# soedinglab/MMseqs2

Measured on AMD Instinct MI355X. Metric: sw_gcells_per_s, higher is better.
Workload: dtype int16

## Files before the change

### mmseqs2_amd/csrc/mmgpu_api.hip

```cpp
#include <algorithm>
#include <atomic>
#include <thread>
#include <cmath>
#include <cstdio>
#include <cstring>
#include <numeric>
#include <string>
#include <vector>

#include "mmgpu_internal.h"

#include <chrono>

using namespace mmgpu;

namespace mmgpu {
thread_local std::string g_last_error;
}
using mmgpu::g_last_error;

extern "C" const char *mmgpu_last_error(void) { return g_last_error.c_str(); }

extern "C" int mmgpu_init(mmgpu_ctx **out, int device_id) {
    if (!out) return fail(MMGPU_ERR_ARG, "mmgpu_init: ctx is NULL");
// ... 594 lines not shown
        hit_out.resize((size_t)total_hits);
    }
    b->h_qout_off.assign(nq + 1, 0);
    if (mode >= MMGPU_SW_START && !pf) b->h_out_target.resize((size_t)total_hits);
    return MMGPU_OK;
}

int SwPrepare::copy_query(uint32_t i, int *qminp) {
    const mmgpu_sw_query &Q = qs[i];
    memcpy(qres.data() + qoff[i], Q.q, Q.qlen);
    int mincb = 0;
    *qminp = minp;
    for (uint32_t k = 0; k < Q.qlen; k++) {
        if (Q.q[k] >= par->alphabet) return fail(MMGPU_ERR_ARG, "mmgpu_sw_prepare: query residue code >= alphabet");
        if (Q.comp_bias && !Q.profile) { qcb[qoff[i] + k] = Q.comp_bias[k]; mincb = std::min<int>(mincb, Q.comp_bias[k]); }
    }
    if (Q.profile) {
        if (Q.profile_letters == 0 || (int)Q.profile_letters > par->alphabet)
            return fail(MMGPU_ERR_ARG, "mmgpu_sw_prepare: profile_letters must be in [1, alphabet]");
        if (qprof.size() + (size_t)par->alphabet * Q.qlen > 0xFFFFFFF0ull) return fail(MMGPU_ERR_UNSUPPORTED, "mmgpu_sw_prepare: more than 4 GB of query profiles in one batch");
        qprof_off[i] = (uint32_t)qprof.size();
        qprof.resize(qprof.size() + (size_t)par->alphabet * Q.qlen, 0);
        const uint32_t rows = std::min<uint32_t>(Q.profile_letters, (uint32_t)par->alphabet - 1);
        memcpy(qprof.data() + qprof_off[i], Q.profile, (size_t)rows * Q.qlen);
        *qminp = 0;
        for (size_t k = 0; k < (size_t)Q.profile_letters * Q.qlen; k++) *qminp = std::min<int>(*qminp, Q.profile[k]);
        b->any_profile = true;
        b->h_query_is_profile.resize(nq, 0);
        b->h_query_is_profile[i] = 1;
    }
    if (!(*qminp + mincb + par->gap_extend > -par->gap_open))
        return fail(MMGPU_ERR_UNSUPPORTED, "mmgpu_sw_prepare: gap penalties too small for this matrix (adjacent insertion+deletion could win)");
    qbias[i] = std::abs(*qminp) + std::abs(mincb);
    qminstart[i] = Q.min_start_score;
    return MMGPU_OK;
}

void SwPrepare::add_rev_jobs(uint32_t query, uint32_t first, uint32_t n, uint32_t shape, uint64_t cells_per_hit) {
    uint64_t per = 6 * JOB_CELLS / std::max<uint64_t>(cells_per_hit, 1);
    per = std::min<uint64_t>(std::max<uint64_t>(per / JOB_ROUND * JOB_ROUND, JOB_ROUND), (uint64_t)SW_REV_JOB_MAX);
    for (uint32_t k = 0; k < n; k += (uint32_t)per) {
        SwJob j;
        j.query = query;
        j.hit_begin = first + k;
        j.hit_end = first + std::min<uint32_t>(k + (uint32_t)per, n);
        j.shape = shape;
        rev_jobs.push_back(j);
        rev_cells.push_back(cells_per_hit * (j.hit_end - j.hit_begin) * 65536u + (n - k));
    }
}

void SwPrepare::add_slot_jobs(uint32_t i, uint32_t shape, uint32_t round, bool multi) {
    const mmgpu_sw_query &Q = qs[i];
    const uint64_t est_cells = (uint64_t)Q.qlen * ((Q.qlen + c->mean_len) / 2 + 1) * round;
    const uint32_t per_job = job_slots(round, JOB_CELLS / est_cells);
    for (uint32_t k = 0; k < pf_stride; k += per_job) {
        SwJob j;
        j.query = i;
        j.hit_begin = hit_cursor + k;
        j.hit_end = hit_cursor + std::min<uint32_t>(k + per_job, pf_stride);
        j.shape = shape | (multi ? n_multi++ << 8 : 0u);
        jobs.push_back(j);
        job_cells.push_back((uint64_t)Q.qlen * (j.hit_end - j.hit_begin) * 65536u + (pf_stride - k));
    }
    if (multi && mode >= MMGPU_SW_START)
        add_rev_jobs(i, hit_cursor, pf_stride, shape, (uint64_t)Q.qlen * ((Q.qlen + c->mean_len) / 2 + 1));
    max_tlen = c->db.max_len;
}

int SwPrepare::copy_queries() {
    for (uint32_t i = 0; i < nq; i++) {
        const mmgpu_sw_query &Q = qs[i];
        if (Q.qlen == 0) {
            b->h_qout_off[i + 1] = out_cursor;
            continue;
        }
        int qminp;
        if (int e = copy_query(i, &qminp)) return e;
        int rpl; bool multi;
        pick_class(Q.qlen, &rpl, &multi);
        any_multi |= multi;
        const uint32_t shape = (multi ? 32u : 0u) + (uint32_t)rpl - 1;
        const int grp = sw_shape_group(shape);
        b->group_lds[grp] = std::max(b->group_lds[grp], sw_lds_bytes(rpl, par->alphabet));
        const uint32_t round = (multi && Q.qlen >= LONG_QUERY) ? JOB_ROUND / 4 : JOB_ROUND;
        const uint32_t n_slots = pf ? pf_stride : Q.n_targets;
        if (pf) add_slot_jobs(i, shape, round, multi);
        else deferred.push_back(Deferred{i, hit_cursor, out_cursor, shape, round, multi});
        hit_cursor += n_slots;
        out_cursor += n_slots;
        b->h_qout_off[i + 1] = out_cursor;
    }
    return MMGPU_OK;
}

void SwPrepare::cut_list_jobs_of(size_t from, size_t to) {
    std::vector<uint32_t> ord;
    for (size_t d = from; d < to; d++) {
        const Deferred &D = deferred[d];
        const mmgpu_sw_query &Q = qs[D.query];
        PerQuery &P = per_query[d];
        const bool same_list = d > from && Q.target_ids == qs[deferred[d - 1].query].target_ids && Q.n_targets == qs[deferred[d - 1].query].n_targets;
        if (!same_list) {
            ord.resize(Q.n_targets);
            std::iota(ord.begin(), ord.end(), 0u);
            for (uint32_t k = 0; k < Q.n_targets; k++)
                if (Q.target_ids[k] >= c->db.n) { P.bad = true; break; }
            if (P.bad) continue;
            std::stable_sort(ord.begin(), ord.end(), [&](uint32_t a, uint32_t bb) {
                return c->h_len[Q.target_ids[a]] > c->h_len[Q.target_ids[bb]];
            });
        }
        for (uint32_t k = 0; k < Q.n_targets; k++) {
            const uint32_t t = Q.target_ids[ord[k]];
            hit_target[D.hit_cursor + k] = t;
            hit_out[D.hit_cursor + k] = D.out_cursor + ord[k];
            P.sum_cells += (uint64_t)Q.qlen * c->h_len[t];
            P.max_tlen = std::max(P.max_tlen, c->h_len[t]);
        }
        for (uint32_t k = 0; k < Q.n_targets;) {
            uint64_t jc = 0;
            uint32_t e = k;
            while (e < Q.n_targets && e - k < JOB_HITS) {
                const uint32_t stop = std::min<uint32_t>(e + D.round, Q.n_targets);
                for (; e < stop; e++) jc += (uint64_t)Q.qlen * c->h_len[hit_target[D.hit_cursor + e]];
                const uint32_t held = e - k;
                if (jc >= JOB_CELLS && (held <= 16 || held % JOB_ROUND == 0)) break;
            }
            SwJob j;
            j.query = D.query;
            j.hit_begin = D.hit_cursor + k;
            j.hit_end = D.hit_cursor + e;
            j.shape = D.shape;
            P.jobs.push_back(j);
            P.cells.push_back(jc);
            k = e;
        }
        if (Q.n_targets) P.rev_mid_len = c->h_len[hit_target[D.hit_cursor + Q.n_targets / 2]];
        if (mode >= MMGPU_SW_START)
            for (uint32_t k = 0; k < Q.n_targets; k++) b->h_out_target[D.out_cursor + k] = Q.target_ids[k];
    }
}

void SwPrepare::cut_list_jobs() {
    per_query.resize(deferred.size());
    static const unsigned host_threads = std::min(16u, std::max(1u, std::thread::hardware_concurrency()));
    const size_t n_thr = std::max<size_t>(1, std::min<size_t>(host_threads, total_hits / 65536 + 1));
    if (n_thr <= 1) {
        cut_list_jobs_of(0, deferred.size());
        return;
    }
    std::vector<std::thread> pool;
    size_t from = 0;
    uint64_t acc = 0;
    const uint64_t share = total_hits / n_thr + 1;
    for (size_t d = 0; d < deferred.size(); d++) {
        acc += qs[deferred[d].query].n_targets;
        if (acc >= share || d + 1 == deferred.size()) {
            pool.emplace_back(&SwPrepare::cut_list_jobs_of, this, from, d + 1);
            from = d + 1;
            acc = 0;
        }
    }
    for (std::thread &t : pool) t.join();
}

int SwPrepare::join_list_jobs() {
// ... 290 lines not shown
    S.n_slots = (uint32_t)slots;
    S.full = b->o_full.as<mmgpu_sw_hit>();
    S.status = b->o_status.as<uint32_t>();
    HIP_TRY(launch_sw_owned_scatter(S, c->stream));
    return MMGPU_OK;
}

}

extern "C" int mmgpu_sw_gather_owned(mmgpu_ctx *c, mmgpu_sw_batch_t *b, const void **d_full, const void **d_status) {
    if (!c || !b) return fail(MMGPU_ERR_ARG, "mmgpu_sw_gather_owned: NULL argument");
    const int n = c->comm ? c->comm->n_ranks : 1;
    for (int attempt = 0; attempt < 2; attempt++) {
        mmgpu::XchgBlock blk[2];
        if (int e = mmgpu::sw_gather_begin(c, b, n, blk)) return e;
        for (int k = 0; k < 2; k++)
            if (int e = mmgpu::comm_allgather(c, blk[k].send, blk[k].recv, blk[k].bytes)) return e;
        if (int e = mmgpu::sw_gather_finish(c, b, n)) return e;
        bool again = false;
        if (n > 1 && attempt == 0)
            if (int e = mmgpu::sw_gather_overflowed(c, b, &again)) return e;
        if (!again) break;
    }
    if (d_full) *d_full = b->o_full.p;
    if (d_status) *d_status = b->o_status.p;
    return MMGPU_OK;
}

extern "C" int mmgpu_sw_fetch_owned(mmgpu_ctx *c, mmgpu_sw_batch_t *b, mmgpu_sw_hit *out, uint32_t *records) {
    if (!c || !b) return fail(MMGPU_ERR_ARG, "mmgpu_sw_fetch_owned: NULL argument");
    if (!b->owned || !b->o_full.p) return fail(MMGPU_ERR_STATE, "mmgpu_sw_fetch_owned: nothing gathered (mmgpu_sw_gather_owned first)");
    HIP_TRY(hipSetDevice(c->device));
    uint32_t st[2] = {0, 0};
    HIP_TRY(hipMemcpyAsync(st, b->o_status.p, 8, hipMemcpyDeviceToHost, c->stream));
    if (out) HIP_TRY(hipMemcpyAsync(out, b->o_full.p, (size_t)b->n_queries * b->o_stride * sizeof(mmgpu_sw_hit), hipMemcpyDeviceToHost, c->stream));
    HIP_TRY(hipStreamSynchronize(c->stream));
    if (records) *records = st[0];
    if (st[1]) return fail(MMGPU_ERR_STATE, "mmgpu_sw_fetch_owned: the send buffer of a rank overflowed (uneven shards); rerun the gather with MMGPU_SW_GATHER_DENSE=1");
    return MMGPU_OK;
}

static int sw_launch_groups(mmgpu_ctx *c, mmgpu_sw_batch_t *b, bool rev_only, const uint8_t *rev_force) {
    if (!c->fork) {
        int prio_low = 0, prio_high = 0;
        HIP_TRY(hipDeviceGetStreamPriorityRange(&prio_low, &prio_high));
        for (int g = 0; g < SW_GROUPS; g++) {
            const int prio = g == SW_GROUPS - 1 ? prio_high : (g == 0 ? prio_low : (prio_low + prio_high) / 2);
            HIP_TRY(hipStreamCreateWithPriority(&c->side[g], hipStreamNonBlocking, prio));
        }
        HIP_TRY(hipEventCreateWithFlags(&c->fork, hipEventDisableTiming));
        for (auto &e : c->join) HIP_TRY(hipEventCreateWithFlags(&e, hipEventDisableTiming));
    }
    HIP_TRY(hipEventRecord(c->fork, c->stream));
    for (int g = 0; g < SW_GROUPS; g++) HIP_TRY(hipStreamWaitEvent(c->side[g], c->fork, 0));
    for (int g = SW_GROUPS - 1; g >= 0; g--) {
        hipStream_t st = c->side[g];
        {
            SwLaunch L;
            L.jobs = b->d_jobs.as<SwJob>() + b->group_begin[g];
            L.n_jobs = b->group_begin[g + 1] - b->group_begin[g];
            L.q_res = b->d_qres.as<uint8_t>();
            L.q_cb = b->d_qcb.as<int8_t>();
            L.q_off = b->d_qoff.as<uint32_t>();
            L.q_bias = b->d_qbias.as<int32_t>();
            L.q_minstart = b->d_qminstart.as<int32_t>();
            L.q_prof = b->any_profile ? b->d_qprof.as<int8_t>() : nullptr;
            L.q_prof_off = b->any_profile ? b->d_qprof_off.as<uint32_t>() : nullptr;
            L.t_res = c->db.res;
            L.t_off4 = c->db.off4;
            L.t_len = c->db.len;
            L.hit_target = b->d_hit_target.as<uint32_t>();
            L.hit_out = b->d_hit_out.as<uint32_t>();
            L.out = b->d_out.as<mmgpu_sw_hit>();
            L.mat = b->d_mat.as<int8_t>();
            L.alphabet = b->alphabet;
            L.gap_open = b->gap_open;
            L.gap_extend = b->gap_extend;
            L.q_hit_count = b->from_pf ? b->d_pf_counts.as<uint32_t>() : nullptr;
            L.hit_stride = b->slot_stride;
            L.scratch = b->d_scratch.as<uint2>();
            L.scratch_cols = b->scratch_cols;
            L.scratch_busy = b->d_scratch_busy.as<uint32_t>();
            L.scratch_slots = std::max<uint32_t>(b->scratch_slots, 1);
            L.rev_mode = rev_only ? 2 : (b->mode == MMGPU_SW_START_NOT_WORD ? 1 : 0);
            L.rev_only = rev_only ? 1 : 0;
            L.rev_force = rev_force;
            HIP_TRY(launch_sw(L, g, b->group_lds[g], b->mode >= MMGPU_SW_START, st));
            if (g == SW_GROUPS - 1 && b->n_rev_jobs && b->mode >= MMGPU_SW_START) {
                SwLaunch Rv = L;
                Rv.jobs = b->d_jobs.as<SwJob>() + b->n_jobs;
                Rv.n_jobs = b->n_rev_jobs;
                HIP_TRY(launch_sw_rev_multi(Rv, b->group_lds[g], st));
            }
            if (getenv("MMGPU_TRACE")) {
                fprintf(stderr, "[sw_run] group %d jobs %u lds %zu both %d from_pf %d scratch_cols %u\n", g, L.n_jobs, b->group_lds[g], (int)(b->mode >= MMGPU_SW_START), (int)b->from_pf, b->scratch_cols);
                fflush(stderr);
                const auto t0 = std::chrono::steady_clock::now();
                hipError_t e = hipStreamSynchronize(st);
                fprintf(stderr, "[sw_run] group %d done after %.2f ms: %s\n", g,
                        std::chrono::duration<double, std::milli>(std::chrono::steady_clock::now() - t0).count(), hipGetErrorString(e));
                fflush(stderr);
            }
        }
    }
    for (int k = 0; k < SW_GROUPS; k++) {
        HIP_TRY(hipEventRecord(c->join[k], c->side[k]));
        HIP_TRY(hipStreamWaitEvent(c->stream, c->join[k], 0));
    }
    return MMGPU_OK;
}

extern "C" int mmgpu_sw_run(mmgpu_ctx *c, mmgpu_sw_batch_t *b) {
    if (!c || !b) return fail(MMGPU_ERR_ARG, "mmgpu_sw_run: NULL argument");
    HIP_TRY(hipSetDevice(c->device));
    hipEvent_t ev0 = nullptr, ev1 = nullptr;
    if (b->events.size() < 256) {
        HIP_TRY(hipEventCreate(&ev0));
        HIP_TRY(hipEventCreate(&ev1));
        b->events.push_back(std::make_pair(ev0, ev1));
        HIP_TRY(hipEventRecord(ev0, c->stream));
    }
    if (int e = sw_launch_groups(c, b, false, nullptr)) return e;
    if (ev1) HIP_TRY(hipEventRecord(ev1, c->stream));
    b->ran = true;
    b->h_res_valid = false;
    return MMGPU_OK;
}

extern "C" int mmgpu_sw_reverse_pairs(mmgpu_ctx *c, mmgpu_sw_batch_t *b, const uint32_t *pair_index, uint32_t n, mmgpu_sw_hit *out) {
    if (!c || !b || (!pair_index && n)) return fail(MMGPU_ERR_ARG, "mmgpu_sw_reverse_pairs: NULL argument");
    if (!b->ran) return fail(MMGPU_ERR_STATE, "mmgpu_sw_reverse_pairs: batch was never run");
    if (b->mode < MMGPU_SW_START) return fail(MMGPU_ERR_STATE, "mmgpu_sw_reverse_pairs: the batch was prepared without a start-position mode");
    if (b->owned) return fail(MMGPU_ERR_UNSUPPORTED, "mmgpu_sw_reverse_pairs: not for batches of owned pairs (sharded runs)");
    if (n == 0) return MMGPU_OK;
    HIP_TRY(hipSetDevice(c->device));
    std::vector<uint8_t> flags((size_t)b->pairs, (uint8_t)0);
    for (uint32_t k = 0; k < n; k++) {
        if (pair_index[k] >= b->pairs) return fail(MMGPU_ERR_ARG, "mmgpu_sw_reverse_pairs: pair index out of range");
        flags[pair_index[k]] = 1;
    }
    DevBuf d_flags;
    d_flags.bind(c->cache);
    HIP_TRY(d_flags.alloc(flags.size()));
    HIP_TRY(hipMemcpyAsync(d_flags.p, flags.data(), flags.size(), hipMemcpyHostToDevice, c->stream));
    if (int e = sw_launch_groups(c, b, true, d_flags.as<uint8_t>())) return e;
    if (out)
        for (uint32_t k = 0; k < n; k++)
            HIP_TRY(hipMemcpyAsync(out + k, b->d_out.as<mmgpu_sw_hit>() + pair_index[k], sizeof(mmgpu_sw_hit), hipMemcpyDeviceToHost, c->stream));
    HIP_TRY(hipStreamSynchronize(c->stream));
    if (b->h_res_valid)
        for (uint32_t k = 0; k < n; k++)
            HIP_TRY(hipMemcpy(&b->h_res[pair_index[k]], b->d_out.as<mmgpu_sw_hit>() + pair_index[k], sizeof(mmgpu_sw_hit), hipMemcpyDeviceToHost));
    return MMGPU_OK;
}

extern "C" int mmgpu_sw_fetch(mmgpu_ctx *c, mmgpu_sw_batch_t *b, mmgpu_sw_hit *out) {
    if (!c || !b || (!out && b->pairs)) return fail(MMGPU_ERR_ARG, "mmgpu_sw_fetch: NULL argument");
    if (!b->ran) return fail(MMGPU_ERR_STATE, "mmgpu_sw_fetch: batch was never run");
    HIP_TRY(hipSetDevice(c->device));
    if (b->pairs)
        HIP_TRY(hipMemcpyAsync(out, b->d_out.p, (size_t)b->pairs * sizeof(mmgpu_sw_hit), hipMemcpyDeviceToHost, c->stream));
    HIP_TRY(hipStreamSynchronize(c->stream));
    return MMGPU_OK;
}

extern "C" int mmgpu_sw_fetch_device(mmgpu_ctx *c, mmgpu_sw_batch_t *b, void *d_out) {
// ... 700 lines not shown
```

### mmseqs2_amd/csrc/mmgpu_internal.h

```cpp
#ifndef MMGPU_INTERNAL_H
#define MMGPU_INTERNAL_H

#include <hip/hip_runtime.h>
#include <stdint.h>
#include <cstdlib>
#include <cstring>

#include <algorithm>
#include <array>
#include <string>
#include <map>
#include <mutex>
#include <chrono>
#include <memory>
#include <vector>
#include <thread>
#include <atomic>

#include "../../include/mmgpu.h"
#include "nucl_core.h"
#include "block_plan.h"

namespace mmgpu {

struct DeviceDb {
    uint8_t *res = nullptr;
    uint32_t *off4 = nullptr;
    uint32_t *len = nullptr;
    uint32_t n = 0;
    uint32_t max_len = 0;
    uint64_t total_residues = 0;
    int alphabet = 0;
    size_t res_bytes = 0;
};

struct SwJob {
    uint32_t query;
    uint32_t hit_begin;
    uint32_t hit_end;
    uint32_t shape;
};

struct SwLaunch {
    const SwJob *jobs;
    uint32_t n_jobs;
    const uint8_t *q_res;
    const int8_t *q_cb;
    const uint32_t *q_off;
    const int32_t *q_bias;
    const int32_t *q_minstart;
    const int8_t *q_prof;
    const uint32_t *q_prof_off;
    const uint8_t *t_res;
    const uint32_t *t_off4;
    const uint32_t *t_len;
    const uint32_t *hit_target;
    const uint32_t *hit_out;
    mmgpu_sw_hit *out;
    const int8_t *mat;
    int alphabet;
    int gap_open, gap_extend;
    uint2 *scratch;
    uint32_t scratch_cols;
    uint32_t *scratch_busy;
    uint32_t scratch_slots;
    const uint32_t *q_hit_count;
    uint32_t hit_stride;
    int rev_mode = 0;
    int rev_only = 0;
    const uint8_t *rev_force = nullptr;
};

constexpr int SW_PF_MAX_LIST = 16384;
constexpr int SW_FROM_PF_STAT_SLOTS = 64;

struct SwFromPfArgs {
    const mmgpu_pf_hit *pf_hits;
    uint32_t pf_stride;
    const uint32_t *hit_count;
    uint32_t stride;
    const uint32_t *q_off;
    const uint32_t *t_len;
    uint32_t *hit_target, *hit_out;
    unsigned long long *cells, *pairs;
    uint32_t *count_copy;
    uint32_t *slot_target;
};

constexpr int SW_REV_JOB_MAX = 1024;
hipError_t launch_sw_rev_multi(const SwLaunch &L, size_t lds_bytes, hipStream_t stream);
hipError_t launch_sw_from_pf(const SwFromPfArgs &A, uint32_t nq, hipStream_t stream);
uint32_t sw_multi_resident_blocks(size_t lds_bytes, bool both_passes, int compute_units);

#ifndef MMGPU_SW_MAX_R
#define MMGPU_SW_MAX_R 28
#endif
constexpr int SW_MAX_R = MMGPU_SW_MAX_R;
static_assert(SW_MAX_R >= 16 && SW_MAX_R <= 32, "multi-tile bodies exist for 8..32 rows per lane: a query cut into tiles gets at least SW_MAX_R / 2");
#ifndef MMGPU_SW_MIN_WAVES
#define MMGPU_SW_MIN_WAVES 2
#endif
constexpr int SW_MIN_WAVES = MMGPU_SW_MIN_WAVES;
#ifndef MMGPU_SW_GROUPS
#define MMGPU_SW_GROUPS 4
#endif
constexpr int SW_GROUPS = MMGPU_SW_GROUPS;
static_assert(SW_GROUPS == 3 || SW_GROUPS == 4, "three or four kernel groups");
int sw_shape_group(uint32_t shape);
hipError_t launch_sw(const SwLaunch &L, int group, size_t lds_bytes, bool both_passes, hipStream_t stream);
size_t sw_lds_bytes(int rows_per_lane, int alphabet);

constexpr int PF_T = 4096;
constexpr int PF_IDS_PER_BIN = 4096;
constexpr int PF_SAT_CAP = 1024;
constexpr int PF_CAND0 = 32;
constexpr int PF_QSTAGE = 2048;
constexpr int PF_MAX_HITS = 4096;
constexpr int PF_MAX_HITS_BIG = 131072;

struct PfList {
    uint32_t start;
    uint32_t len;
    uint32_t lprefix;
    uint32_t pos;
};

struct PfCand {
    uint32_t id;
    uint32_t arr;
    uint32_t score;
    uint16_t diag;
    uint16_t pad;
};

__host__ __device__ inline uint32_t pf_el_count(uint32_t s) { return (s & 0x80000000u) ? ((s >> 23) & 0xFFu) : (s < 255u ? s : 255u); }
__host__ __device__ inline uint32_t pf_el_exact(uint32_t s) { return (s & 0x80000000u) ? (s & 0x7FFFFFu) : s; }

constexpr int PF_PROW = 32;
constexpr int PF_PROF_LETTERS = 20;

struct PfKmerArgs {
    const uint8_t *q_res;
    const int16_t *q_thr;
    uint32_t n_pos;
    uint8_t pat[16];
    uint32_t kalph, n3;
    uint32_t kbase;
    const int16_t *s3;
    const uint32_t *i3;
    const uint32_t *offsets;
    const uint32_t *nonempty;
    const uint4 *cofs;
    const uint16_t *cum3;
    uint32_t cum_w;
    int32_t score_min;
    int k;
    const int16_t *s2;
    const uint32_t *i2;
    const uint16_t *cum2;
    uint32_t cum2_w;
    int32_t score2_min;
    const uint8_t *q_kind;
    const int16_t *prof_score;
    const uint8_t *prof_letter;
    int exact;
    const uint32_t *order;
    uint32_t *nsim;
    const uint32_t *list_base;
    PfList *lists;
    uint32_t *pos_entries;
};

struct PfSplitArgs {
    const uint32_t *tile_q, *tile_idx;
    const uint32_t *q_off;
    const uint32_t *q_entries;
    const uint32_t *pos_entry_base;
    const uint32_t *list_base;
    const PfList *lists;
    const uint64_t *idx_entries;
    uint32_t bins;
    uint32_t *split;
    uint8_t *split_hi;
    uint16_t *bin_off;
    uint32_t *bucket_count;
};

struct PfDedupArgs {
    uint32_t n_queries, bins;
    uint32_t q_first;
    uint32_t cand_origin;
    const uint32_t *q_tile_base, *q_ntiles;
    const uint32_t *split;
// ... 624 lines not shown
```

### mmseqs2_amd/csrc/sw_kernel.hip

```cpp
#include "mmgpu_internal.h"

namespace mmgpu {

namespace {

constexpr int GROUP = 16;
constexpr int WAVES = 4;
constexpr int GROUPS_PER_WAVE = 64 / GROUP;
constexpr int HITS_PER_WAVE = 2 * GROUPS_PER_WAVE;
constexpr unsigned NEG2 = 0x80008000u;

typedef short s16x2 __attribute__((ext_vector_type(2)));
typedef unsigned short u16x2 __attribute__((ext_vector_type(2)));

__device__ __forceinline__ unsigned pk_add_sat(unsigned a, unsigned b) {
    return __builtin_bit_cast(unsigned, __builtin_elementwise_add_sat(__builtin_bit_cast(s16x2, a),
                                                                      __builtin_bit_cast(s16x2, b)));
}
__device__ __forceinline__ unsigned pk_max_s(unsigned a, unsigned b) {
    return __builtin_bit_cast(unsigned, __builtin_elementwise_max(__builtin_bit_cast(s16x2, a),
                                                                  __builtin_bit_cast(s16x2, b)));
}
__device__ __forceinline__ unsigned pk_max_u(unsigned a, unsigned b) {
    return __builtin_bit_cast(unsigned, __builtin_elementwise_max(__builtin_bit_cast(u16x2, a),
                                                                  __builtin_bit_cast(u16x2, b)));
}
__device__ __forceinline__ unsigned pk_sub_sat_u(unsigned a, unsigned b) {
    return __builtin_bit_cast(unsigned, __builtin_elementwise_sub_sat(__builtin_bit_cast(u16x2, a),
                                                                      __builtin_bit_cast(u16x2, b)));
}
__device__ __forceinline__ unsigned bfi(unsigned mask, unsigned a, unsigned b) {
    return (a & mask) | (b & ~mask);
}
__device__ __forceinline__ unsigned from_lane_above(unsigned head, unsigned v) {
    return __builtin_amdgcn_update_dpp(head, v, 0x111 , 0xF, 0xF, false);
}

#ifndef MMGPU_SW_PREFETCH
#define MMGPU_SW_PREFETCH 1
#endif
#define SW_KEEP_IN_ROW(x) asm volatile("" : "+v"(x))

__host__ __device__ constexpr int lane_stride_bytes(int R) {
    int slots = (R * 2 + 15) / 16;
    if ((slots & 1) == 0) slots += 1;
    return slots * 16;
}

template <int R>
struct Tile {
    static constexpr int ROWS = GROUP * R;
    static constexpr int LANE_STRIDE = lane_stride_bytes(R);
    static constexpr int ROW_STRIDE = GROUP * LANE_STRIDE;
};

template <int R, bool REV>
__device__ __forceinline__ void build_profile(unsigned char *lds, const uint8_t *q, const int8_t *cb, int qlen,
                                              int tile_base, const int8_t *mat, int alphabet, const int8_t *prof) {
    using T = Tile<R>;
    const int total = (alphabet + 1) * T::ROWS;
    for (int idx = threadIdx.x; idx < total; idx += blockDim.x) {
        const int letter = idx / T::ROWS;
        const int row = idx - letter * T::ROWS;
        const int rg = tile_base + row;
        short v = (short)-32768;
        if (letter < alphabet && rg < qlen) {
            const int qi = REV ? (qlen - 1 - rg) : rg;
            v = prof ? (short)prof[letter * qlen + qi] : (short)((int)mat[letter * alphabet + q[qi]] + (int)cb[qi]);
        }
        const int lane = row / R, r = row - lane * R;
        *reinterpret_cast<short *>(lds + letter * T::ROW_STRIDE + lane * T::LANE_STRIDE + r * 2) = v;
    }
}

__device__ __forceinline__ bool sw_rev_wanted(const SwLaunch &L, uint32_t slot, int min_start) {
    const mmgpu_sw_hit &f = L.out[slot];
    const int s = f.score;
    if (L.rev_mode == 2) return s > 0 && L.rev_force[slot] != 0;
    return s > 0 && s >= min_start && !(L.rev_mode == 1 && f.word != 0);
}

constexpr int SW_REV_JOB_HITS = 1024;
static_assert(SW_REV_JOB_HITS == SW_REV_JOB_MAX, "host and kernel disagree on the reverse job size");
constexpr int SW_LDS_HEADER = SW_REV_JOB_HITS * 2 + 64;

template <int R, bool MULTI, bool REV, bool PF>
__device__ __forceinline__ void sw_body(const SwLaunch &L, const SwJob job) {
    using T = Tile<R>;
    extern __shared__ __attribute__((aligned(16))) unsigned char lds_all[];
    uint16_t *live = reinterpret_cast<uint16_t *>(lds_all);
    uint32_t *live_wave = reinterpret_cast<uint32_t *>(lds_all + SW_REV_JOB_HITS * 2);
    uint32_t *next_chunk = reinterpret_cast<uint32_t *>(lds_all + SW_REV_JOB_HITS * 2 + 16);
    unsigned char *lds = lds_all + SW_LDS_HEADER;
    if (MULTI) __builtin_amdgcn_s_setprio(3);
    const int lane = threadIdx.x & 63;
    const int wave = __builtin_amdgcn_readfirstlane(threadIdx.x >> 6);
    const int g = lane & (GROUP - 1);
    const int grp = lane / GROUP;

    const uint32_t qbeg = L.q_off[job.query];
    const int qlen = (int)(L.q_off[job.query + 1] - qbeg);
    const uint8_t *q = L.q_res + qbeg;
    const int8_t *cb = L.q_cb + qbeg;
    const int qbias = L.q_bias[job.query];
    const int8_t *prof = nullptr;
    if (L.q_prof_off) {
        const uint32_t po = L.q_prof_off[job.query];
        if (po != 0xFFFFFFFFu) prof = L.q_prof + po;
    }
    const int n_tiles = MULTI ? (qlen + T::ROWS - 1) / T::ROWS : 1;

    const unsigned go2 = (unsigned)L.gap_open * 0x10001u;
    const unsigned ge2 = (unsigned)L.gap_extend * 0x10001u;
    const unsigned pad_letter = (unsigned)L.alphabet;

    if (threadIdx.x == 0) *next_chunk = 0;
    if (!MULTI && !REV) {
        build_profile<R, REV>(lds, q, cb, qlen, 0, L.mat, L.alphabet, prof);
        __syncthreads();
    }

    uint32_t n_hits = job.hit_end - job.hit_begin;
    if (REV) {
        const int min_start = L.q_minstart[job.query];
        uint32_t total = 0;
        for (uint32_t base = 0; base < n_hits; base += WAVES * 64) {
            const uint32_t idx = base + threadIdx.x;
            bool pass = false;
            if (idx < n_hits) pass = sw_rev_wanted(L, L.hit_out[job.hit_begin + idx], min_start);
            const unsigned long long bal = __ballot(pass);
            if (lane == 0) live_wave[wave] = (uint32_t)__popcll(bal);
            __syncthreads();
            uint32_t before = 0, round_total = 0;
#pragma unroll
            for (int w = 0; w < WAVES; ++w) {
                const uint32_t c = live_wave[w];
                before += w < wave ? c : 0u;
                round_total += c;
            }
            if (pass) live[total + before + (uint32_t)__popcll(bal & ((1ull << lane) - 1ull))] = (uint16_t)idx;
            total += round_total;
            __syncthreads();
        }
        n_hits = total;
        if (n_hits == 0) return;
        if (!MULTI) {
            build_profile<R, REV>(lds, q, cb, qlen, 0, L.mat, L.alphabet, prof);
            __syncthreads();
        }
    }
    const uint32_t n_iter = (n_hits + WAVES * HITS_PER_WAVE - 1) / (WAVES * HITS_PER_WAVE);

    for (uint32_t it = 0; !MULTI || it < n_iter; ++it) {
        uint32_t chunk = it * WAVES + wave;
        if (!MULTI) {
            if (lane == 0) chunk = atomicAdd(next_chunk, 1u);
            chunk = __builtin_amdgcn_readfirstlane(chunk);
        }
        const uint32_t slot0 = chunk * HITS_PER_WAVE;
        if (!MULTI && slot0 >= n_hits) break;

        const uint32_t sA = slot0 + grp * 2, sB = sA + 1;
        const bool vA = sA < n_hits, vB = sB < n_hits;
        const uint32_t hA = job.hit_begin + (REV ? (uint32_t)live[vA ? sA : 0] : sA);
        const uint32_t hB = job.hit_begin + (REV ? (uint32_t)live[vB ? sB : 0] : sB);
        const uint32_t tA = vA ? L.hit_target[hA] : 0u, tB = vB ? L.hit_target[hB] : 0u;
        const uint8_t *pA = L.t_res + (size_t)L.t_off4[tA] * 4;
        const uint8_t *pB = L.t_res + (size_t)L.t_off4[tB] * 4;
        int colsA = vA ? (int)L.t_len[tA] : 0, colsB = vB ? (int)L.t_len[tB] : 0;
        int r0A = 0, r0B = 0;
        int endA = 0, endB = 0;
        unsigned rev_target = 0xFFFFFFFFu;
        if (REV) {
            mmgpu_sw_hit fa, fb;
            fa.score = 0; fa.q_end = 0; fa.t_end = 0;
            fb = fa;
            if (vA) fa = L.out[L.hit_out[hA]];
            if (vB) fb = L.out[L.hit_out[hB]];
            colsA = vA ? fa.t_end + 1 : 0;
            colsB = vB ? fb.t_end + 1 : 0;
            endA = colsA > 0 ? fa.t_end : 0;
            endB = colsB > 0 ? fb.t_end : 0;
            r0A = colsA > 0 ? qlen - 1 - fa.q_end : 0;
            r0B = colsB > 0 ? qlen - 1 - fb.q_end : 0;
            rev_target = (colsA > 0 ? (unsigned)fa.score & 0xFFFFu : 0xFFFFu) | ((colsB > 0 ? (unsigned)fb.score & 0xFFFFu : 0xFFFFu) << 16);
        }
        int ncols = colsA > colsB ? colsA : colsB;
        ncols = max(ncols, __shfl_xor(ncols, 16));
        ncols = max(ncols, __shfl_xor(ncols, 32));
        ncols = __builtin_amdgcn_readfirstlane(ncols);
        const int nsteps = ncols + GROUP - 1;

        unsigned long long bestA = 0, bestB = 0;

        uint2 *scr = nullptr;
        if (MULTI) scr = L.scratch + ((size_t)((job.shape >> 8) * WAVES + wave) * GROUPS_PER_WAVE + grp) * 2 * L.scratch_cols;

        for (int tile = 0; tile < n_tiles; ++tile) {
            const int tile_base = tile * T::ROWS;
            if (MULTI) {
                __syncthreads();
                build_profile<R, REV>(lds, q, cb, qlen, tile_base, L.mat, L.alphabet, prof);
                __syncthreads();
            }
            const uint2 *scr_in = MULTI ? scr + (size_t)((tile + 1) & 1) * L.scratch_cols : nullptr;
            uint2 *scr_out = MULTI ? scr + (size_t)(tile & 1) * L.scratch_cols : nullptr;
            const bool has_above = MULTI && tile > 0;
            const bool has_below = MULTI && tile + 1 < n_tiles;

            unsigned Hp[R], E[R], aux[R];
#pragma unroll
            for (int r = 0; r < R; ++r) { Hp[r] = 0; E[r] = 0; aux[r] = 0; }
            if (REV) {
#pragma unroll
                for (int r = 0; r < R; ++r) {
                    const int rg = tile_base + g * R + r;
                    aux[r] = (rg >= r0A ? 0xFFFFu : 0u) | (rg >= r0B ? 0xFFFF0000u : 0u);
                }
            }
            unsigned vmax = 0, bestcol = 0xFFFFFFFFu;
            unsigned rev_rowA = 0, rev_rowB = 0;
            unsigned Hup_prev = 0;
            unsigned out_H = 0, out_F = 0;

            auto letters4 = [&](const uint8_t *p, int end, int k) -> unsigned {
                if (!REV) return reinterpret_cast<const unsigned *>(p)[k];
                int o = end - 3 - 4 * k;
                o = o < -3 ? -3 : o;
                unsigned w;
                __builtin_memcpy(&w, p + o, 4);
                return w;
            };
            unsigned wA = letters4(pA, endA, 0), wB = letters4(pB, endB, 0);
            unsigned wA_next = letters4(pA, endA, 1), wB_next = letters4(pB, endB, 1);
#ifndef MMGPU_SW_UP_DEPTH
#define MMGPU_SW_UP_DEPTH 4
#endif
            constexpr int UPD = MMGPU_SW_UP_DEPTH;
            uint2 up[UPD];
#pragma unroll
            for (int k = 0; k < UPD; ++k) up[k] = make_uint2(0, 0);
            if (has_above) {
                const int last = ncols - 1 < 0 ? 0 : ncols - 1;
#pragma unroll
                for (int k = 0; k < UPD; ++k) up[k] = scr_in[min(k, last)];
            }

            constexpr int ND = (R + 1) / 2;
            unsigned pav_next[PF ? ND : 1], pbv_next[PF ? ND : 1];
            auto load_rows = [&](unsigned letters, unsigned *pav, unsigned *pbv) {
                const unsigned a = letters & 0xFFu, b = (letters >> 8) & 0xFFu;
                const uint4 *rowA = reinterpret_cast<const uint4 *>(lds + a * T::ROW_STRIDE + g * T::LANE_STRIDE);
                const uint4 *rowB = reinterpret_cast<const uint4 *>(lds + b * T::ROW_STRIDE + g * T::LANE_STRIDE);
#pragma unroll
                for (int k = 0; k < ND / 4; ++k) {
                    const uint4 pa = rowA[k], pb = rowB[k];
                    pav[4 * k] = pa.x; pav[4 * k + 1] = pa.y; pav[4 * k + 2] = pa.z; pav[4 * k + 3] = pa.w;
                    pbv[4 * k] = pb.x; pbv[4 * k + 1] = pb.y; pbv[4 * k + 2] = pb.z; pbv[4 * k + 3] = pb.w;
                }
                if constexpr (ND % 4 >= 2) {
                    const uint2 pa = *reinterpret_cast<const uint2 *>(rowA + ND / 4);
                    const uint2 pb = *reinterpret_cast<const uint2 *>(rowB + ND / 4);
                    pav[(ND / 4) * 4] = pa.x; pav[(ND / 4) * 4 + 1] = pa.y;
                    pbv[(ND / 4) * 4] = pb.x; pbv[(ND / 4) * 4 + 1] = pb.y;
                }
                if constexpr (ND % 2 == 1) {
                    pav[ND - 1] = reinterpret_cast<const unsigned *>(rowA)[ND - 1];
                    pbv[ND - 1] = reinterpret_cast<const unsigned *>(rowB)[ND - 1];
                }
            };
            unsigned let = pad_letter * 0x101u;
            auto head_letters = [&](int c, int j) -> unsigned {
                const unsigned sh = (unsigned)(REV ? 3 - j : j) * 8u;
                const unsigned la0 = __builtin_amdgcn_ubfe(wA, sh, 8u);
                const unsigned lb0 = __builtin_amdgcn_ubfe(wB, sh, 8u);
                return (c < colsA ? la0 : pad_letter) | ((c < colsB ? lb0 : pad_letter) << 8);
            };
            if (PF) {
                let = from_lane_above(head_letters(0, 0), let);
                load_rows(let, pav_next, pbv_next);
            }

            for (int s0 = PF ? -1 : 0; s0 < nsteps; s0 += 4) {
            const int jn = min(4, nsteps - s0);
#pragma nounroll
            for (int j = PF && s0 < 0 ? 1 : 0; j < jn; ++j) {
                const int s = s0 + j;
                unsigned head_let = 0;
                if (!PF) head_let = head_letters(s, j);
                const unsigned Hup = from_lane_above(up[0].x, out_H);
                unsigned f = from_lane_above(up[0].y, out_F);
                if (!PF) let = from_lane_above(head_let, let);
                if (has_above) {
#pragma unroll
                    for (int k = 0; k + 1 < UPD; ++k) up[k] = up[k + 1];
                    int c = s + UPD; if (c > ncols - 1) c = ncols - 1; if (c < 0) c = 0;
                    up[UPD - 1] = scr_in[c];
                }
                unsigned pav[ND], pbv[ND];
                if (PF) {
#pragma unroll
                    for (int k = 0; k < ND; ++k) { pav[k] = pav_next[k]; pbv[k] = pbv_next[k]; }
                } else {
                    load_rows(let, pav, pbv);
                }

                unsigned hd = Hup_prev;
                Hup_prev = Hup;
                unsigned cmax = 0;
                unsigned pre[R], es[R];
#pragma unroll
                for (int r = 0; r < R; ++r) {
                    unsigned P = __builtin_amdgcn_perm(pbv[r / 2], pav[r / 2], (r & 1) ? 0x07060302u : 0x05040100u);
                    if (REV) P = __builtin_amdgcn_bitop3_b32(aux[r], P, NEG2, 0xCA);
                    pre[r] = pk_max_s(pk_add_sat(r == 0 ? hd : Hp[r - 1], P), E[r]);
                    es[r] = pk_sub_sat_u(E[r], ge2);
                }
                if (PF) {
                    let = from_lane_above(head_letters(s + 1, j), let);
                    load_rows(let, pav_next, pbv_next);
                }
#pragma unroll
                for (int r = 0; r < R; ++r) {
                    const unsigned h = pk_max_s(pre[r], f);
                    const unsigned fs = pk_sub_sat_u(f, ge2);
                    const unsigned t = pk_sub_sat_u(h, go2);
                    cmax = pk_max_u(cmax, h);
                    if (MULTI) SW_KEEP_IN_ROW(cmax);
                    f = pk_max_u(fs, t);
                    E[r] = pk_max_u(es[r], t);
                    SW_KEEP_IN_ROW(E[r]);
                    Hp[r] = h;
                }
                out_H = Hp[R - 1];
                out_F = f;

// ... 238 lines not shown
            cells += (unsigned long long)qlen * len;
        }
        key[k] = v;
    }
    __syncthreads();
    const uint32_t base = q * A.stride;
    if (n <= 512) {
        for (uint32_t i = threadIdx.x; i < n; i += 256) {
            const uint32_t mine = key[i];
            uint32_t r = 0;
            for (uint32_t j = 0; j < n; j++) r += key[j] < mine ? 1u : 0u;
            A.hit_target[base + r] = hits[i].id;
            A.hit_out[base + r] = base + i;
            A.slot_target[base + i] = hits[i].id;
            if (r == 0) atomicMax(stat + 2, (unsigned long long)(0xFFFFu - (mine >> 16)));
        }
    } else {
    for (uint32_t size = 2; size <= np2; size <<= 1) {
        for (uint32_t stride = size >> 1; stride > 0; stride >>= 1) {
            for (uint32_t k = threadIdx.x; k < np2 / 2; k += 256) {
                const uint32_t i = 2 * k - (k & (stride - 1));
                const uint32_t j = i + stride;
                const bool up = (i & size) == 0;
                const uint32_t a = key[i], b = key[j];
                if ((a > b) == up) {
                    key[i] = b;
                    key[j] = a;
                }
            }
            __syncthreads();
        }
    }
    for (uint32_t r = threadIdx.x; r < n; r += 256) {
        const uint32_t k = key[r] & 0xFFFFu;
        A.hit_target[base + r] = hits[k].id;
        A.hit_out[base + r] = base + k;
        A.slot_target[base + r] = hits[r].id;
    }
    if (threadIdx.x == 0 && n) atomicMax(stat + 2, (unsigned long long)(0xFFFFu - (key[0] >> 16)));
    }
    for (uint32_t r = n + threadIdx.x; r < A.stride; r += 256) {
        A.hit_target[base + r] = 0;
        A.hit_out[base + r] = base + r;
        A.slot_target[base + r] = 0;
    }
    if (threadIdx.x == 0) A.count_copy[q] = n;
    for (int d = 1; d < 64; d <<= 1) cells += __shfl_xor(cells, d);
    if ((threadIdx.x & 63u) == 0 && cells) atomicAdd(stat, cells);
    if (threadIdx.x == 0 && n) atomicAdd(stat + 1, (unsigned long long)n);
}

}

hipError_t launch_sw_from_pf(const SwFromPfArgs &A, uint32_t nq, hipStream_t stream) {
    static_assert((SW_PF_MAX_LIST & (SW_PF_MAX_LIST - 1)) == 0 && (size_t)SW_PF_MAX_LIST * sizeof(uint32_t) <= 65536,
                  "SW_PF_MAX_LIST: a power of two whose dwords fit 64 KB of dynamic LDS");
    if (A.stride > (uint32_t)SW_PF_MAX_LIST) return hipErrorInvalidValue;
    if (nq == 0) return hipSuccess;
    uint32_t np2 = 1;
    while (np2 < A.stride) np2 <<= 1;
    const size_t lds = (size_t)np2 * sizeof(uint32_t);
    if (lds > 65536) return hipErrorInvalidValue;
    const hipError_t attr = hipFuncSetAttribute(reinterpret_cast<const void *>(sw_from_pf_kernel),
                                                hipFuncAttributeMaxDynamicSharedMemorySize, 65536);
    if (attr != hipSuccess) return attr;
    hipLaunchKernelGGL(sw_from_pf_kernel, dim3(nq), dim3(256), lds, stream, A);
    return hipGetLastError();
}

uint32_t sw_multi_resident_blocks(size_t lds_bytes, bool both_passes, int compute_units) {
    int per_cu = 0;
    const size_t lds = lds_bytes + SW_LDS_HEADER;
    hipError_t e = both_passes ? hipOccupancyMaxActiveBlocksPerMultiprocessor(&per_cu, sw_kernel<SW_GROUPS - 1, true>, WAVES * 64, lds)
                               : hipOccupancyMaxActiveBlocksPerMultiprocessor(&per_cu, sw_kernel<SW_GROUPS - 1, false>, WAVES * 64, lds);
    if (e == hipSuccess && both_passes) {
        int rev = 0;
        if (hipOccupancyMaxActiveBlocksPerMultiprocessor(&rev, sw_rev_multi_kernel, WAVES * 64, lds) == hipSuccess) per_cu = std::max(per_cu, rev);
    }
    if (e != hipSuccess || per_cu < 1) per_cu = 8;
    per_cu = per_cu + 1 > 8 ? 8 : per_cu + 1;
    return (uint32_t)per_cu * (uint32_t)(compute_units > 0 ? compute_units : 256);
}

size_t sw_lds_bytes(int rows_per_lane, int alphabet) {
    return (size_t)(alphabet + 1) * GROUP * lane_stride_bytes(rows_per_lane);
}

hipError_t launch_sw_rev_multi(const SwLaunch &L, size_t lds_bytes, hipStream_t stream) {
    if (L.n_jobs == 0) return hipSuccess;
    hipLaunchKernelGGL(sw_rev_multi_kernel, dim3(L.n_jobs), dim3(WAVES * 64), lds_bytes + SW_LDS_HEADER, stream, L);
    return hipGetLastError();
}

int sw_shape_group(uint32_t shape) {
    if (shape >= 32) return SW_GROUPS - 1;
    const int R = (int)shape + 1;
    return R <= 12 ? 0 : (R <= 24 ? 1 : 2);
}

hipError_t launch_sw(const SwLaunch &L, int group, size_t lds_bytes, bool both_passes, hipStream_t stream) {
    static_assert(GROUP == 16, "the shape codes assume 16-lane groups");
    if (L.n_jobs == 0) return hipSuccess;
    dim3 grid(L.n_jobs), block(WAVES * 64);
    const size_t lds = lds_bytes + SW_LDS_HEADER;
    switch (group * 2 + (both_passes ? 1 : 0)) {
        case 0: hipLaunchKernelGGL((sw_kernel<0, false>), grid, block, lds, stream, L); break;
        case 1: hipLaunchKernelGGL((sw_kernel<0, true>), grid, block, lds, stream, L); break;
        case 2: hipLaunchKernelGGL((sw_kernel<1, false>), grid, block, lds, stream, L); break;
        case 3: hipLaunchKernelGGL((sw_kernel<1, true>), grid, block, lds, stream, L); break;
        case 4: hipLaunchKernelGGL((sw_kernel<2, false>), grid, block, lds, stream, L); break;
        case 5: hipLaunchKernelGGL((sw_kernel<2, true>), grid, block, lds, stream, L); break;
        case 6: hipLaunchKernelGGL((sw_kernel<SW_GROUPS - 1, false>), grid, block, lds, stream, L); break;
        case 7: hipLaunchKernelGGL((sw_kernel<SW_GROUPS - 1, true>), grid, block, lds, stream, L); break;
        default: return hipErrorInvalidValue;
    }
    return hipGetLastError();
}

void warm_sw() {
    hipFuncAttributes a;
    (void)hipFuncGetAttributes(&a, reinterpret_cast<const void *>(&sw_rev_multi_kernel));
}

}
```

Measured before the change: 4436.

## Keep all query-profile tiles resident in LDS for short multi-tile queries

For multi-tile queries whose full set of per-tile score profiles fits in a 64 KB LDS budget, every tile profile is built once up front and kept resident. This removes the per-tile, per-iteration profile rebuild and the barriers around it. Because the workgroup no longer syncs between tiles, it also switches to dynamic atomic chunk scheduling like single-tile jobs. The cost is a larger LDS allocation per group, which may lower occupancy for the multi-tile kernel group.

Result: faster. 4511 (median of 6 runs) (+1.7%).

```diff
diff --git a/mmseqs2_amd/csrc/mmgpu_api.hip b/mmseqs2_amd/csrc/mmgpu_api.hip
--- a/mmseqs2_amd/csrc/mmgpu_api.hip
+++ b/mmseqs2_amd/csrc/mmgpu_api.hip
@@ -700,7 +700,8 @@
         any_multi |= multi;
         const uint32_t shape = (multi ? 32u : 0u) + (uint32_t)rpl - 1;
         const int grp = sw_shape_group(shape);
-        b->group_lds[grp] = std::max(b->group_lds[grp], sw_lds_bytes(rpl, par->alphabet));
+        const uint32_t held = multi && sw_multi_resident(sw_tiles(Q.qlen, rpl), rpl, par->alphabet, SW_RESIDENT_LDS) ? sw_tiles(Q.qlen, rpl) : 1u;
+        b->group_lds[grp] = std::max(b->group_lds[grp], (size_t)held * sw_profile_bytes(rpl, par->alphabet));
         const uint32_t round = (multi && Q.qlen >= LONG_QUERY) ? JOB_ROUND / 4 : JOB_ROUND;
         const uint32_t n_slots = pf ? pf_stride : Q.n_targets;
         if (pf) add_slot_jobs(i, shape, round, multi);
@@ -1157,6 +1158,7 @@
             L.scratch_cols = b->scratch_cols;
             L.scratch_busy = b->d_scratch_busy.as<uint32_t>();
             L.scratch_slots = std::max<uint32_t>(b->scratch_slots, 1);
+            L.resident_lds = SW_RESIDENT_LDS;
             L.rev_mode = rev_only ? 2 : (b->mode == MMGPU_SW_START_NOT_WORD ? 1 : 0);
             L.rev_only = rev_only ? 1 : 0;
             L.rev_force = rev_force;
diff --git a/mmseqs2_amd/csrc/mmgpu_internal.h b/mmseqs2_amd/csrc/mmgpu_internal.h
--- a/mmseqs2_amd/csrc/mmgpu_internal.h
+++ b/mmseqs2_amd/csrc/mmgpu_internal.h
@@ -64,6 +64,7 @@
     uint32_t scratch_cols;
     uint32_t *scratch_busy;
     uint32_t scratch_slots;
+    uint32_t resident_lds = 0;
     const uint32_t *q_hit_count;
     uint32_t hit_stride;
     int rev_mode = 0;
@@ -108,7 +109,27 @@
 static_assert(SW_GROUPS == 3 || SW_GROUPS == 4, "three or four kernel groups");
 int sw_shape_group(uint32_t shape);
 hipError_t launch_sw(const SwLaunch &L, int group, size_t lds_bytes, bool both_passes, hipStream_t stream);
-size_t sw_lds_bytes(int rows_per_lane, int alphabet);
+
+constexpr int SW_LDS_HEADER = SW_REV_JOB_MAX * 2 + 64;
+__host__ __device__ constexpr int lane_stride_bytes(int R) {
+    int slots = (R * 2 + 15) / 16;
+    if ((slots & 1) == 0) slots += 1;
+    return slots * 16;
+}
+__host__ __device__ constexpr uint32_t sw_profile_bytes(int R, int alphabet) {
+    return (uint32_t)(alphabet + 1) * 16u * (uint32_t)lane_stride_bytes(R);
+}
+#ifndef MMGPU_SW_RESIDENT_LDS
+#define MMGPU_SW_RESIDENT_LDS 65536
+#endif
+constexpr uint32_t SW_RESIDENT_LDS = MMGPU_SW_RESIDENT_LDS;
+static_assert(SW_RESIDENT_LDS <= 65536u, "a workgroup asks for at most 64 KB of dynamic LDS");
+__host__ __device__ constexpr uint32_t sw_tiles(uint32_t qlen, int R) { return (qlen + 16u * (uint32_t)R - 1u) / (16u * (uint32_t)R); }
+__host__ __device__ constexpr bool sw_multi_resident(uint32_t n_tiles, int R, int alphabet, uint32_t budget) {
+    return (unsigned long long)n_tiles * sw_profile_bytes(R, alphabet) + (unsigned long long)SW_LDS_HEADER <= (unsigned long long)budget;
+}
+static_assert(sw_multi_resident(2, 28, 21, 65536) && sw_multi_resident(3, 24, 21, 65536) && !sw_multi_resident(3, 25, 21, 65536) &&
+              !sw_multi_resident(4, 22, 21, 65536) && !sw_multi_resident(2, 8, 21, 0), "residency rule");
 
 constexpr int PF_T = 4096;
 constexpr int PF_IDS_PER_BIN = 4096;
diff --git a/mmseqs2_amd/csrc/sw_kernel.hip b/mmseqs2_amd/csrc/sw_kernel.hip
--- a/mmseqs2_amd/csrc/sw_kernel.hip
+++ b/mmseqs2_amd/csrc/sw_kernel.hip
@@ -40,12 +40,6 @@
 #define MMGPU_SW_PREFETCH 1
 #endif
 #define SW_KEEP_IN_ROW(x) asm volatile("" : "+v"(x))
-
-__host__ __device__ constexpr int lane_stride_bytes(int R) {
-    int slots = (R * 2 + 15) / 16;
-    if ((slots & 1) == 0) slots += 1;
-    return slots * 16;
-}
 
 template <int R>
 struct Tile {
@@ -53,6 +47,7 @@
     static constexpr int LANE_STRIDE = lane_stride_bytes(R);
     static constexpr int ROW_STRIDE = GROUP * LANE_STRIDE;
 };
+static_assert(GROUP == 16, "sw_profile_bytes and sw_tiles (mmgpu_internal.h) assume 16-lane groups");
 
 template <int R, bool REV>
 __device__ __forceinline__ void build_profile(unsigned char *lds, const uint8_t *q, const int8_t *cb, int qlen,
@@ -82,7 +77,7 @@
 
 constexpr int SW_REV_JOB_HITS = 1024;
 static_assert(SW_REV_JOB_HITS == SW_REV_JOB_MAX, "host and kernel disagree on the reverse job size");
-constexpr int SW_LDS_HEADER = SW_REV_JOB_HITS * 2 + 64;
+static_assert(SW_LDS_HEADER == SW_REV_JOB_HITS * 2 + 64, "the header holds the live hits and the scheduling words");
 
 template <int R, bool MULTI, bool REV, bool PF>
 __device__ __forceinline__ void sw_body(const SwLaunch &L, const SwJob job) {
@@ -108,7 +103,15 @@
         const uint32_t po = L.q_prof_off[job.query];
         if (po != 0xFFFFFFFFu) prof = L.q_prof + po;
     }
-    const int n_tiles = MULTI ? (qlen + T::ROWS - 1) / T::ROWS : 1;
+    const int n_tiles = MULTI ? (int)sw_tiles((uint32_t)qlen, R) : 1;
+    const uint32_t tile_bytes = sw_profile_bytes(R, L.alphabet);
+    const bool resident = MULTI && sw_multi_resident((uint32_t)n_tiles, R, L.alphabet, L.resident_lds);
+    const bool dynamic = !MULTI || resident;
+    auto build_all_tiles = [&]() {
+        for (int tile = 0; tile < n_tiles; ++tile)
+            build_profile<R, REV>(lds + (uint32_t)tile * tile_bytes, q, cb, qlen, tile * T::ROWS, L.mat, L.alphabet, prof);
+        __syncthreads();
+    };
 
     const unsigned go2 = (unsigned)L.gap_open * 0x10001u;
     const unsigned ge2 = (unsigned)L.gap_extend * 0x10001u;
@@ -119,6 +122,7 @@
         build_profile<R, REV>(lds, q, cb, qlen, 0, L.mat, L.alphabet, prof);
         __syncthreads();
     }
+    if (MULTI && !REV && resident) build_all_tiles();
 
     uint32_t n_hits = job.hit_end - job.hit_begin;
     if (REV) {
@@ -148,17 +152,18 @@
             build_profile<R, REV>(lds, q, cb, qlen, 0, L.mat, L.alphabet, prof);
             __syncthreads();
         }
+        if (MULTI && resident) build_all_tiles();
     }
     const uint32_t n_iter = (n_hits + WAVES * HITS_PER_WAVE - 1) / (WAVES * HITS_PER_WAVE);
 
-    for (uint32_t it = 0; !MULTI || it < n_iter; ++it) {
+    for (uint32_t it = 0; dynamic || it < n_iter; ++it) {
         uint32_t chunk = it * WAVES + wave;
-        if (!MULTI) {
+        if (dynamic) {
             if (lane == 0) chunk = atomicAdd(next_chunk, 1u);
             chunk = __builtin_amdgcn_readfirstlane(chunk);
         }
         const uint32_t slot0 = chunk * HITS_PER_WAVE;
-        if (!MULTI && slot0 >= n_hits) break;
+        if (dynamic && slot0 >= n_hits) break;
 
         const uint32_t sA = slot0 + grp * 2, sB = sA + 1;
         const bool vA = sA < n_hits, vB = sB < n_hits;
@@ -198,11 +203,12 @@
 
         for (int tile = 0; tile < n_tiles; ++tile) {
             const int tile_base = tile * T::ROWS;
-            if (MULTI) {
+            if (MULTI && !resident) {
                 __syncthreads();
                 build_profile<R, REV>(lds, q, cb, qlen, tile_base, L.mat, L.alphabet, prof);
                 __syncthreads();
             }
+            const unsigned char *const lds_tile = MULTI && resident ? lds + (uint32_t)tile * tile_bytes : lds;
             const uint2 *scr_in = MULTI ? scr + (size_t)((tile + 1) & 1) * L.scratch_cols : nullptr;
             uint2 *scr_out = MULTI ? scr + (size_t)(tile & 1) * L.scratch_cols : nullptr;
             const bool has_above = MULTI && tile > 0;
@@ -250,8 +256,8 @@
             unsigned pav_next[PF ? ND : 1], pbv_next[PF ? ND : 1];
             auto load_rows = [&](unsigned letters, unsigned *pav, unsigned *pbv) {
                 const unsigned a = letters & 0xFFu, b = (letters >> 8) & 0xFFu;
-                const uint4 *rowA = reinterpret_cast<const uint4 *>(lds + a * T::ROW_STRIDE + g * T::LANE_STRIDE);
-                const uint4 *rowB = reinterpret_cast<const uint4 *>(lds + b * T::ROW_STRIDE + g * T::LANE_STRIDE);
+                const uint4 *rowA = reinterpret_cast<const uint4 *>(lds_tile + a * T::ROW_STRIDE + g * T::LANE_STRIDE);
+                const uint4 *rowB = reinterpret_cast<const uint4 *>(lds_tile + b * T::ROW_STRIDE + g * T::LANE_STRIDE);
 #pragma unroll
                 for (int k = 0; k < ND / 4; ++k) {
                     const uint4 pa = rowA[k], pb = rowB[k];
@@ -656,10 +662,6 @@
     return (uint32_t)per_cu * (uint32_t)(compute_units > 0 ? compute_units : 256);
 }
 
-size_t sw_lds_bytes(int rows_per_lane, int alphabet) {
-    return (size_t)(alphabet + 1) * GROUP * lane_stride_bytes(rows_per_lane);
-}
-
 hipError_t launch_sw_rev_multi(const SwLaunch &L, size_t lds_bytes, hipStream_t stream) {
     if (L.n_jobs == 0) return hipSuccess;
     hipLaunchKernelGGL(sw_rev_multi_kernel, dim3(L.n_jobs), dim3(WAVES * 64), lds_bytes + SW_LDS_HEADER, stream, L);
```
